# manycore-research/PlankAssembly

Hardware: AMD Instinct MI355X
Metric: train samples/sec (fwd+bwd+all-reduce+Adam), d_model=512 seq=1024 [value: bf16 MFMA, f32 accumulate / master weights; train.f32 / train.x3: the same step in exact f32 / f32 with bf16x3 products = the parity paths] (higher is better)
Workload: dtype bf16; 1 GPU; train_complete.yaml model d_model=512 H=8 dff=1024 6+6 post-norm layers, dropout 0.2, S=1024 (MAX_INPUT_LENGTH 1025), T=128, batch 16/GPU; global_batch=16, seq_len=1024, parallelism=dp1

## Files before the change

### plankassembly_amd/csrc/gemm.hip

```cpp
#include <stdlib.h>
#include <atomic>
#include <new>
#include <mutex>
#include <vector>
#include <type_traits>
#include <utility>
#include "pa_device.h"
#include <mutex>
#include <vector>
#include "../../include/plank_hip.h"
#include "gemm_common.h"

namespace {

constexpr int BM = 128, BN = 128, NT = 256;
__device__ __attribute__((aligned(16))) const uint32_t pa_zero16[4] = {0u, 0u, 0u, 0u};
typedef short s16x4 __attribute__((ext_vector_type(4)));

#ifdef PA_GEMM_TRACE
__device__ unsigned long long pa_trace[8192];
__device__ int pa_trace_n;
#define TR_DECL __shared__ unsigned long long tr_lds[1024]; int tr_n = 0
#define TR(tag) do { if (blockIdx.x == 0 && threadIdx.x == 0 && tr_n < 1022) { tr_lds[tr_n++] = (unsigned long long)(tag); tr_lds[tr_n++] = __builtin_amdgcn_s_memtime(); } } while (0)
#define TR_FLUSH do { if (blockIdx.x == 0 && threadIdx.x == 0) { for (int i_ = 0; i_ < tr_n; ++i_) pa_trace[i_] = tr_lds[i_]; pa_trace_n = tr_n; } } while (0)
// ... 1503 lines not shown
#ifndef PA_G3S_OLD
    u32x4 F[8];
#pragma unroll
    for (int s_ = 0; s_ < 4; ++s_) { PA_RD128(F[2 * s_], lds0 + fa_off + xs[s_]); PA_RD128(F[2 * s_ + 1], lds0 + fb_off + xs[s_]); }
#pragma unroll 1
    while (true) {
        const bool has_next = pending >= 2;
        if (has_next) wait_items(pending - 2);
        __builtin_amdgcn_s_barrier();
        if (cd_u < p.units) issue();
        {
            const uint32_t nst = lds0 + ((sc + 1) & (NSTG - 1)) * STAGE;
#pragma unroll
            for (int s_ = 0; s_ < 4; ++s_) {
                asm volatile("s_waitcnt lgkmcnt(6)" : "+v"(F[2 * s_]), "+v"(F[2 * s_ + 1]));
                acc = __builtin_amdgcn_mfma_f32_32x32x16_bf16(*reinterpret_cast<const bf16x8*>(&F[2 * s_ + 1]), *reinterpret_cast<const bf16x8*>(&F[2 * s_]), acc, 0, 0, 0);
                PA_RD128(F[2 * s_], nst + fa_off + xs[s_]); PA_RD128(F[2 * s_ + 1], nst + fb_off + xs[s_]);
            }
        }
        sc = (sc + 1) & (NSTG - 1);
        if (++cc_t >= nt) {
            PA_TR3(3);
            epilogue(cun);
#ifdef PA_GEMM_TRACE3
            PA_TR3(5);
            asm volatile("s_waitcnt vmcnt(0)" ::: "memory");
#endif
            PA_TR3(4);
            cc_u += ustride; cc_t = 0;
            if (cc_u < p.units) unit_of(cc_u, cun);
        }
        --pending;
        if (!has_next) break;
    }
    asm volatile("s_waitcnt lgkmcnt(0)" : "+v"(F[0]), "+v"(F[1]), "+v"(F[2]), "+v"(F[3]), "+v"(F[4]), "+v"(F[5]), "+v"(F[6]), "+v"(F[7]));
#else
    u32x4 F0[2], F1[2];
    frag(F0, lds0, 0);
    auto item = [&](auto HOT_) -> bool {
        constexpr bool HOT = decltype(HOT_)::value;
        const uint32_t st = lds0 + sc * STAGE;
        __builtin_amdgcn_s_barrier();
        if constexpr (!HOT) { if (cd_u < p.units) issue(); }
        wait_frag(F0); acc = __builtin_amdgcn_mfma_f32_32x32x16_bf16(*reinterpret_cast<const bf16x8*>(&F0[1]), *reinterpret_cast<const bf16x8*>(&F0[0]), acc, 0, 0, 0);
        frag(F1, st, 1); if constexpr (HOT) { fetch_q(sd, Q0{}); fetch_q(sd, Q1{}); }
        wait_frag(F1); acc = __builtin_amdgcn_mfma_f32_32x32x16_bf16(*reinterpret_cast<const bf16x8*>(&F1[1]), *reinterpret_cast<const bf16x8*>(&F1[0]), acc, 0, 0, 0);
        frag(F0, st, 2); if constexpr (HOT) { fetch_q(sd, Q2{}); fetch_q(sd, Q3{}); fetch_done(); sd = (sd + 1) & (NSTG - 1); ++cd_t; }
        wait_frag(F0); acc = __builtin_amdgcn_mfma_f32_32x32x16_bf16(*reinterpret_cast<const bf16x8*>(&F0[1]), *reinterpret_cast<const bf16x8*>(&F0[0]), acc, 0, 0, 0);
        frag(F1, st, 3);
        const bool has_next = HOT || pending >= 2;
        wait_frag(F1);
        if (has_next) {
            if constexpr (HOT) wait_items(2); else wait_items(pending - 2);
            __builtin_amdgcn_s_barrier();
            frag(F0, lds0 + ((sc + 1) & (NSTG - 1)) * STAGE, 0);
        }
        acc = __builtin_amdgcn_mfma_f32_32x32x16_bf16(*reinterpret_cast<const bf16x8*>(&F1[1]), *reinterpret_cast<const bf16x8*>(&F1[0]), acc, 0, 0, 0);
        sc = (sc + 1) & (NSTG - 1);
        if constexpr (HOT) { ++cc_t; return true; }
        else {
            if (++cc_t >= nt) {
                PA_TR3(3);
                epilogue(cun);
#ifdef PA_GEMM_TRACE3
                PA_TR3(5);
                asm volatile("s_waitcnt vmcnt(0)" ::: "memory");
#endif
                PA_TR3(4);
                cc_u += ustride; cc_t = 0;
                if (cc_u < p.units) unit_of(cc_u, cun);
            }
            --pending;
            return has_next;
        }
    };
#pragma unroll 1
    while (true) {
        int hot = (pending == 3 && cd_u == cc_u) ? (nt - cd_t - 1) : 0;
#pragma unroll 1
        for (; hot > 0; --hot) item(std::true_type{});
        if (!item(std::false_type{})) break;
    }
#endif
#undef PA_RD128
}

template <int FM, int FN>
__global__ __launch_bounds__(NT, 1) void gemm3w_kernel(GemmP p) {
    using T = bf16;
    constexpr int TBM = 64 * FM, TBN = 64 * FN;
    constexpr int RB = 128, NCH = 8;
    constexpr int A_BYTES = TBM * RB, B_BYTES = TBN * RB;
    constexpr int NLA = TBM * NCH / NT, NLB = TBN * NCH / NT, NLD = NLA + NLB;
    constexpr int NSTG = 3, STAGE = A_BYTES + B_BYTES, EPI = 32 * 32 * 4;
    static_assert(NSTG * STAGE + 4 * EPI <= 160 * 1024, "LDS budget");
    __shared__ __attribute__((aligned(256))) char smem[NSTG * STAGE + 4 * EPI];
    const int tid = threadIdx.x, lane = tid & 63;
    const int wave = __builtin_amdgcn_readfirstlane(tid >> 6);
    const int wm = wave >> 1, wn = wave & 1;
    const int half = lane >> 5;
    constexpr int esz = 2;
    f32x16 acc[FN][FM];
#pragma unroll
    for (int i = 0; i < FN; ++i)
#pragma unroll
        for (int j = 0; j < FM; ++j)
#pragma unroll
            for (int r = 0; r < 16; ++r) acc[i][j][r] = 0.f;

    uint32_t offA[NLA], offB[NLB];
    const char* kA = nullptr; const char* kB = nullptr;
    auto setup = [&](const Unit& un) {
        kA = reinterpret_cast<const char*>(p.A) + (size_t)un.b * p.sA * esz;
        kB = reinterpret_cast<const char*>(p.B) + (size_t)un.b * p.sB * esz;
        const int m0 = un.tile_m * TBM, n0 = un.tile_n * TBN;
#pragma unroll
        for (int i = 0; i < NLA; ++i) {
            const int pidx = tid + i * NT, row = pidx / NCH, ch = ((pidx % NCH) ^ (row / 2)) & (NCH - 1);
            offA[i] = (uint32_t)min(m0 + row, p.M - 1) * (uint32_t)(p.lda * esz) + ch * 16;
        }
#pragma unroll
        for (int i = 0; i < NLB; ++i) {
            const int pidx = tid + i * NT, row = pidx / NCH, ch = ((pidx % NCH) ^ (row / 2)) & (NCH - 1);
            offB[i] = (uint32_t)min(n0 + row, p.N - 1) * (uint32_t)(p.ldb * esz) + ch * 16;
        }
    };
    auto fetch_c = [&](int stage, auto C_) {
        constexpr int c = decltype(C_)::value;
        char* lx = smem + stage * STAGE + (c < NLA ? 0 : A_BYTES);
        constexpr int i = c < NLA ? c : c - NLA;
        const char* src = (c < NLA) ? kA + offA[i] : kB + offB[i];
        __builtin_amdgcn_global_load_lds((const __attribute__((address_space(1))) void*)src,
            (__attribute__((address_space(3))) void*)(lx + (i * NT + wave * 64) * 16), 16, 0, 0);
    };
    auto fetch_done = [&]() { kA += 64 * esz; kB += 64 * esz; };
    auto fetch_range = [&](int stage, auto LO_, auto HI_) {
        constexpr int LO = decltype(LO_)::value, HI = decltype(HI_)::value;
        static_for<LO, HI>([&](auto I_) { fetch_c(stage, I_); });
    };
    auto fetch = [&](int stage) {
        fetch_range(stage, std::integral_constant<int, 0>{}, std::integral_constant<int, NLD>{});
        fetch_done();
    };

    const uint32_t lds0 = (uint32_t)(uintptr_t)((__attribute__((address_space(3))) char*)smem);
    const int sw = ((lane & 31) >> 1) & 7;
    uint32_t xs[4];
#pragma unroll
    for (int s_ = 0; s_ < 4; ++s_) xs[s_] = (uint32_t)((((2 * s_ + half) ^ sw) & 7) << 4);
    const uint32_t fa_off = (wm * 32 * FM + (lane & 31)) * RB, fb_off = (wn * 32 * FN + (lane & 31)) * RB + A_BYTES;
#define PA_RD128O(dst, addr, OFF) asm volatile("ds_read_b128 %0, %1 offset:%2" : "=v"(dst) : "v"(addr), "n"(OFF))
    auto rd1 = [&](u32x4 (&f)[FM + FN], uint32_t st, int s_, auto W_) {
        constexpr int W = decltype(W_)::value;
        if constexpr (W < FM) { const uint32_t ad = st + fa_off + xs[s_]; PA_RD128O(f[W], ad, W * 32 * RB); }
        else { const uint32_t ad = st + fb_off + xs[s_]; PA_RD128O(f[W], ad, (W - FM) * 32 * RB); }
    };
    auto frag = [&](u32x4 (&f)[FM + FN], uint32_t st, int s_) {
        static_for<0, FM + FN>([&](auto I_) { rd1(f, st, s_, I_); });
    };
    auto wait_frag = [&](u32x4 (&f)[FM + FN]) {
        asm volatile("s_waitcnt lgkmcnt(0)" ::: "memory");
#pragma unroll
        for (int i = 0; i < FM + FN; ++i) asm volatile("" : "+v"(f[i]));
    };

    auto epilogue = [&](const Unit& un) {
// ... 926 lines not shown
                const size_t slab = (size_t)a->M * a->N * sizeof(float);
                if (hipMemsetAsync(static_cast<char*>(a->ws) + (size_t)got * slab, 0, (size_t)(want - got) * slab,
                                   reinterpret_cast<hipStream_t>(stream)) != hipSuccess) return PA_EINVAL;
            }
            return 0;
        }
        static const bool dbg_split = getenv("PA_SPLIT_DEBUG") && atoi(getenv("PA_SPLIT_DEBUG"));
        if (dbg_split) fprintf(stderr, "[pa_gemm x3 declined] M %d N %d K %d batch %d akc %d bkc %d lda %d ldb %d sA %lld sB %lld splitk %d aux %d ldaux %d\n",
                               a->M, a->N, a->K, a->batch, a->a_kcontig, a->b_kcontig, a->lda, a->ldb, (long long)a->sA, (long long)a->sB, a->splitk, a->aux ? 1 : 0, a->ldaux);
    }
    if (g_rec) { std::lock_guard<std::mutex> lk(g_rec_mu); if (g_rec) g_rec->push_back(*a); }
    if (a->M <= 0 || a->N <= 0 || a->K <= 0 || a->batch <= 0) return PA_EINVAL;
    if (a->in_dtype != PA_F32 && a->in_dtype != PA_BF16) return PA_EINVAL;
    if (a->out_dtype != PA_F32 && a->out_dtype != PA_BF16) return PA_EINVAL;
    if (a->drop_p < 0.f || a->drop_p >= 1.f) return PA_EINVAL;
    hipStream_t st = reinterpret_cast<hipStream_t>(stream);
    GemmP p;
    p.A = a->A; p.B = a->B; p.C = a->C; p.bias = a->bias; p.R = a->R; p.aux = a->aux;
    p.M = a->M; p.N = a->N; p.K = a->K;
    p.lda = a->lda; p.ldb = a->ldb; p.ldc = a->ldc; p.ldr = a->ldr; p.ldaux = a->ldaux;
    p.sA = a->sA; p.sB = a->sB; p.sC = a->sC; p.sR = a->sR; p.sAux = a->sAux; p.sBias = a->sBias;
    p.batch = a->batch;
    p.alpha = a->alpha; p.relu = a->relu; p.aux_scale = a->aux_scale;
    p.drop_thr = (uint32_t)((double)a->drop_p * 4294967296.0);
    p.drop_scale = (float)(1.0 / (1.0 - (double)p.drop_thr / 4294967296.0));
    p.drop_seed = a->drop_seed;
    p.out_dtype = a->out_dtype;
    p.ln_u = nullptr; p.ln_gamma = nullptr; p.ln_beta = nullptr; p.ln_y = nullptr; p.ldy = 0; p.ln_eps = 0.f;
    p.c_lp = a->C_lp; p.ldc_lp = a->ldc_lp; p.ln_zf = nullptr; p.ldzf = 0; p.ln_y_f32 = 0;
    if (a->C_lp && (a->out_dtype != PA_F32 || a->ldc_lp < a->N || a->ldc_lp % 4 || (reinterpret_cast<uintptr_t>(a->C_lp) & 7))) return PA_EINVAL;
    static const int dbg_bk = getenv("PA_GEMM_BK") ? atoi(getenv("PA_GEMM_BK")) : 64;
    const bool bk32 = a->in_dtype == PA_BF16 && dbg_bk == 32;
    const int BK = a->in_dtype == PA_BF16 ? (bk32 ? 32 : 64) : 16;
    const int nt = (a->K + BK - 1) / BK;
    int splitk = a->splitk > 1 ? a->splitk : 1;
    if (splitk > nt) splitk = nt;
    splitk = (nt + (nt + splitk - 1) / splitk - 1) / ((nt + splitk - 1) / splitk);
    if (splitk > 1 && !a->ws) return PA_EINVAL;
    p.splitk = splitk;
    p.tiles_per_slice = (nt + splitk - 1) / splitk;
    p.tiles_m = (a->M + BM - 1) / BM;
    p.tiles_n = (a->N + BN - 1) / BN;
    p.plain_order = p.tiles_m < 8;
    p.tiles_m_pad = p.plain_order ? p.tiles_m : (p.tiles_m + 7) / 8 * 8;
    p.units = p.tiles_m_pad * p.tiles_n * a->batch * splitk;
    GemmP pk = p;
    if (splitk > 1) { pk.C = a->ws; pk.ldc = a->N; }
    {
        const int osz = (splitk > 1 || a->out_dtype == PA_F32) ? 4 : 2, isz = a->in_dtype == PA_BF16 ? 2 : 4;
        auto ok = [](const void* q, long long ld, long long sb, int esz) {
            return !q || (((reinterpret_cast<uintptr_t>(q) * 1) % (4 * esz) == 0) && (ld % 4 == 0) && (sb % 4 == 0));
        };
        pk.vec_ok = ok(pk.C, pk.ldc, splitk > 1 ? (long long)a->M * a->N : a->sC, osz) && ok(a->R, a->ldr, a->sR, osz) &&
                    ok(a->aux, a->ldaux, a->sAux, isz) && ok(a->bias, 4, a->sBias, 4);
    }
    const int cus = cus_for_gemm();
    static const int dbg_noglds = getenv("PA_GEMM_NOGLDS") ? atoi(getenv("PA_GEMM_NOGLDS")) : 0;
    static const int dbg_grid = getenv("PA_GEMM_GRID") ? atoi(getenv("PA_GEMM_GRID")) :
                                (getenv("PA_GEMM_NST") && atoi(getenv("PA_GEMM_NST")) == 1 ? 1024 : (bk32 ? 768 : 512));
    static const int dbg_bits = getenv("PA_GEMM_DBG") ? atoi(getenv("PA_GEMM_DBG")) : 0;
    pk.dbg = dbg_bits; p.dbg = dbg_bits;
    const int pair_cap = dbg_grid > 0 ? (dbg_grid / 256) * cus + dbg_grid % 256 : 0;
    int grid_x = (pair_cap > 0 && pk.units > pair_cap) ? pair_cap : pk.units;
    dim3 grid(grid_x);
    const bool glds = ((a->K % BK) == 0 || (!a->a_kcontig && !a->b_kcontig && a->in_dtype == PA_BF16 && !bk32)) && !dbg_noglds;
    int rc;
    static const int use_v3 = getenv("PA_GEMM_V3") ? atoi(getenv("PA_GEMM_V3")) : 1;
    const bool v3_layout_ok = (a->a_kcontig && a->b_kcontig) ? (a->K % 64 == 0) : ((!a->a_kcontig || a->K % 64 == 0) && (!a->b_kcontig || a->K % 64 == 0));
    const int valid_units = p.tiles_m * p.tiles_n * a->batch * splitk;
    const bool go_v3 = use_v3 && (valid_units <= 256 || use_v3 == 2) && a->in_dtype == PA_BF16 && !bk32 && !dbg_noglds && is_aligned<bf16>(a) && v3_layout_ok;
    static const int use_small = getenv("PA_GEMM_SMALL") ? atoi(getenv("PA_GEMM_SMALL")) : 1;
    static const int small_max = getenv("PA_GEMM_SMALL_MAX") ? atoi(getenv("PA_GEMM_SMALL_MAX")) : 128;
    static const int small_max_k512 = getenv("PA_GEMM_SMALL_MAX_K512") ? atoi(getenv("PA_GEMM_SMALL_MAX_K512")) : 192;
    const bool go_small = go_v3 && use_small && a->a_kcontig && a->b_kcontig && splitk == 1 && a->K % 64 == 0 &&
                          (valid_units <= small_max || (valid_units <= small_max_k512 && a->K <= 512));
    static const int use_wide = getenv("PA_GEMM_WIDE") ? atoi(getenv("PA_GEMM_WIDE")) : 2;
    const long long wide_tiles = (long long)((a->M + 127) / 128) * ((a->N + 255) / 256) * a->batch;
    const bool go_wide = use_v3 && use_wide && (use_wide == 1 || wide_tiles <= cus) && a->in_dtype == PA_BF16 && !bk32 && !dbg_noglds &&
                         is_aligned<bf16>(a) && a->a_kcontig && a->b_kcontig && splitk == 1 && a->K % 64 == 0 && a->N >= 1024 && valid_units > 256;
    static const int use_tall = getenv("PA_GEMM_TALL") ? atoi(getenv("PA_GEMM_TALL")) : 0;
    const int tall_units = ((a->M + 191) / 192) * ((a->N + 127) / 128) * a->batch;
    const bool go_tall = use_v3 && use_tall && !go_wide && a->in_dtype == PA_BF16 && !bk32 && !dbg_noglds && is_aligned<bf16>(a) && a->a_kcontig &&
                         a->b_kcontig && splitk == 1 && a->K % 64 == 0 && valid_units > 256 && tall_units <= cus;
    static const int use_skinny = getenv("PA_GEMM_SKINNY") ? atoi(getenv("PA_GEMM_SKINNY")) : 2;
    static const int skinny_rows = getenv("PA_GEMM_SKINNY_ROWS") ? atoi(getenv("PA_GEMM_SKINNY_ROWS")) : 512;
    static const int skinny_rows32 = getenv("PA_GEMM_SKINNY_ROWS_F32") ? atoi(getenv("PA_GEMM_SKINNY_ROWS_F32"))
                                     : getenv("PA_GEMM_SKINNY_ROWS") ? atoi(getenv("PA_GEMM_SKINNY_ROWS")) : 2048;
    const int sk_ch = a->in_dtype == PA_BF16 ? 512 : 256;
    const bool go_skinny = use_skinny && (a->in_dtype == PA_F32 || use_skinny >= 2) && a->a_kcontig && a->b_kcontig && splitk == 1 &&
                           a->batch == 1 && a->M <= (a->in_dtype == PA_F32 ? skinny_rows32 : skinny_rows) && a->K % sk_ch == 0 && !a->aux && a->drop_p == 0.f && !dbg_noglds &&
                           (a->in_dtype == PA_BF16 ? is_aligned<bf16>(a) : is_aligned<float>(a));
    static const int use_big = getenv("PA_GEMM_BIG") ? atoi(getenv("PA_GEMM_BIG")) : 0;
    static const int big_minm = getenv("PA_GEMM_BIG_MINM") ? atoi(getenv("PA_GEMM_BIG_MINM")) : 4096;
    static const int big_minn = getenv("PA_GEMM_BIG_MINN") ? atoi(getenv("PA_GEMM_BIG_MINN")) : 256;
    const bool go_big = use_big && !go_skinny && a->in_dtype == PA_BF16 && !dbg_noglds && is_aligned<bf16>(a) && a->a_kcontig && a->b_kcontig &&
                        splitk == 1 && a->K % 64 == 0 && a->M >= big_minm && a->N >= big_minn;
    if (go_big) {
        if (g_rec) { std::lock_guard<std::mutex> lk(g_rec_mu); if (g_rec && g_rec_kind) g_rec_kind->push_back(PA_GEMM_KIND_BIG); if (g_rec && g_rec_group) g_rec_group->push_back(-1); }
        static const int force_tn = getenv("PA_GEMM_BIG_TN") ? atoi(getenv("PA_GEMM_BIG_TN")) : 0;
        int tn = a->N >= 1024 ? 256 : 128;
        const int tm8 = (a->M + 255) / 256;
        if (use_big >= 2) {
            long best = -1;
            for (int w : {256, 192, 128}) {
                const long blocks = (long)tm8 * ((a->N + w - 1) / w) * a->batch;
                const long rounds = (blocks + cus - 1) / cus;
                const long cost = rounds * w * 1000 + ((a->N + w - 1) / w * w - a->N);
                if (best < 0 || cost < best) { best = cost; tn = w; }
            }
        }
        if (force_tn == 256 || force_tn == 192 || force_tn == 128) tn = force_tn;
        GemmP pb = pk;
        pb.tiles_m = tm8; pb.tiles_n = (a->N + tn - 1) / tn;
        pb.plain_order = pb.tiles_m < 8;
        pb.tiles_m_pad = pb.plain_order ? pb.tiles_m : (pb.tiles_m + 7) / 8 * 8;
        pb.units = pb.tiles_m_pad * pb.tiles_n * a->batch;
        const int gb = pb.units < cus ? pb.units : cus;
        if (tn == 256) PA_LAUNCH((gemm8_kernel<4, 2, 2, 4, 64, 2>), dim3(gb), dim3(512), 0, st, pb);
        else if (tn == 192) PA_LAUNCH((gemm8_kernel<4, 2, 2, 3, 64, 2>), dim3(gb), dim3(512), 0, st, pb);
        else PA_LAUNCH((gemm8_kernel<4, 2, 2, 2, 64, 2>), dim3(gb), dim3(512), 0, st, pb);
        return 0;
    }
    if (a->C_lp && !go_skinny) return PA_EINVAL;
    if (go_skinny) {
        if (g_rec) { std::lock_guard<std::mutex> lk(g_rec_mu); if (g_rec && g_rec_kind) g_rec_kind->push_back(PA_GEMM_KIND_SKINNY); if (g_rec && g_rec_group) g_rec_group->push_back(-1); }
        GemmP ps = pk;
        ps.tiles_m = (a->M + SK_T - 1) / SK_T; ps.tiles_n = (a->N + SK_T - 1) / SK_T;
        const dim3 gsk(ps.tiles_m * ps.tiles_n);
        if (a->in_dtype == PA_BF16) PA_LAUNCH((gemm_skinny_kernel<bf16, false>), gsk, dim3(256), 0, st, ps);
        else PA_LAUNCH((gemm_skinny_kernel<float, false>), gsk, dim3(256), 0, st, ps);
        return 0;
    }
    if (g_rec) { std::lock_guard<std::mutex> lk(g_rec_mu); if (g_rec && g_rec_kind) g_rec_kind->push_back((go_wide || go_tall) ? PA_GEMM_KIND_WIDE : (go_small ? PA_GEMM_KIND_SMALL : (go_v3 ? PA_GEMM_KIND_RING : PA_GEMM_KIND_PAIR))); if (g_rec && g_rec_group) g_rec_group->push_back(-1); }
    if (go_wide) {
        GemmP pw = pk;
        pw.tiles_m = (a->M + 127) / 128; pw.tiles_n = (a->N + 255) / 256;
        pw.tiles_m_pad = (pw.tiles_m + 7) / 8 * 8; pw.plain_order = 0;
        pw.units = pw.tiles_m_pad * pw.tiles_n * a->batch;
        const int gw = pw.units < cus ? pw.units : cus;
        PA_LAUNCH((gemm3w_kernel<2, 4>), dim3(gw), dim3(NT), 0, st, pw);
        return 0;
    }
    if (go_tall) {
        GemmP pw = pk;
        pw.tiles_m = (a->M + 191) / 192; pw.tiles_n = (a->N + 127) / 128;
        pw.plain_order = pw.tiles_m < 8;
        pw.tiles_m_pad = pw.plain_order ? pw.tiles_m : (pw.tiles_m + 7) / 8 * 8;
        pw.units = pw.tiles_m_pad * pw.tiles_n * a->batch;
        const int gw = pw.units < cus ? pw.units : cus;
        PA_LAUNCH((gemm3w_kernel<3, 2>), dim3(gw), dim3(NT), 0, st, pw);
        return 0;
    }
    if (go_small) {
        GemmP ps = pk;
        ps.tiles_m = (a->M + 63) / 64; ps.tiles_n = (a->N + 63) / 64; ps.tiles_m_pad = ps.tiles_m; ps.plain_order = 1;
        ps.units = ps.tiles_m * ps.tiles_n * a->batch;
        const int gs = ps.units < 2 * cus ? ps.units : 2 * cus;
        PA_LAUNCH(gemm3s_kernel, dim3(gs), dim3(NT), 0, st, ps);
        rc = 0;
    } else
    if (go_v3) {
        const int g3 = pk.units < cus ? pk.units : cus;
        if (a->a_kcontig && a->b_kcontig) PA_LAUNCH((gemm3_kernel<true, true, GemmP>), dim3(g3), dim3(NT), 0, st, pk);
        else if (a->a_kcontig) PA_LAUNCH((gemm3_kernel<true, false, GemmP>), dim3(g3), dim3(NT), 0, st, pk);
        else if (a->b_kcontig) PA_LAUNCH((gemm3_kernel<false, true, GemmP>), dim3(g3), dim3(NT), 0, st, pk);
        else PA_LAUNCH((gemm3_kernel<false, false, GemmP>), dim3(g3), dim3(NT), 0, st, pk);
        rc = 0;
    } else
    if (a->in_dtype == PA_BF16) {
        if (bk32) rc = launch_layout<bf16, 32, 3>(pk, a->a_kcontig, a->b_kcontig, is_aligned<bf16>(a), glds, grid, st);
        else rc = launch_layout<bf16, 64, 2>(pk, a->a_kcontig, a->b_kcontig, is_aligned<bf16>(a), glds, grid, st);
    } else {
        rc = launch_layout<float, 16, 2>(pk, a->a_kcontig, a->b_kcontig, is_aligned<float>(a), glds, grid, st);
    }
    if (rc) return rc;
    if (splitk > 1 && a->splitk_defer) {
        if (a->out_dtype != PA_F32 || a->bias || a->R || a->aux || a->relu || a->drop_p > 0.f || a->alpha != 1.f || a->batch != 1) return PA_EINVAL;
        return 0;
    }
    if (splitk > 1) {
        size_t total = (size_t)a->batch * a->M * a->N;
        int blocks = (int)((total + 255) / 256);
        if (blocks > 2048) blocks = 2048;
        if (a->in_dtype == PA_BF16)
            PA_LAUNCH(splitk_reduce_kernel<bf16>, dim3(blocks), dim3(256), 0, st, p, (const float*)a->ws);
        else
            PA_LAUNCH(splitk_reduce_kernel<float>, dim3(blocks), dim3(256), 0, st, p, (const float*)a->ws);
    }
    return 0;
}

namespace {
template <typename TW>
__global__ __launch_bounds__(256) void ln_fold_weights_kernel(TW* Wf, float* u, float* v, const float* W, const float* bias,
                                                              const float* gamma, const float* beta, int N, int K) {
    __shared__ float red[2][4];
    const int n = blockIdx.x;
    float su = 0.f, sv = 0.f;
    for (int k = threadIdx.x; k < K; k += 256) {
        const float w = W[(size_t)n * K + k];
        const TW wf = (TW)(w * gamma[k]);
        Wf[(size_t)n * K + k] = wf;
        su += (float)wf;
        sv += w * beta[k];
    }
    su = wave_sum(su); sv = wave_sum(sv);
    if ((threadIdx.x & 63) == 0) { red[0][threadIdx.x >> 6] = su; red[1][threadIdx.x >> 6] = sv; }
    __syncthreads();
    if (threadIdx.x == 0) {
        u[n] = (red[0][0] + red[0][1]) + (red[0][2] + red[0][3]);
        v[n] = (bias ? bias[n] : 0.f) + (red[1][0] + red[1][1]) + (red[1][2] + red[1][3]);
    }
}
}
extern "C" int pa_ln_fold_weights(void* Wf, float* u, float* v, const float* W, const float* bias, const float* gamma,
                                  const float* beta, int32_t N, int32_t K, void* stream) {
    if (!Wf || !u || !v || !W || !gamma || !beta || N <= 0 || K <= 0) return PA_EINVAL;
    PA_LAUNCH(ln_fold_weights_kernel<bf16>, dim3(N), dim3(256), 0, reinterpret_cast<hipStream_t>(stream), (bf16*)Wf, u, v, W, bias, gamma, beta, N, K);
    return 0;
}
extern "C" int pa_ln_fold_weights_f32(float* Wf, float* u, float* v, const float* W, const float* bias, const float* gamma,
                                      const float* beta, int32_t N, int32_t K, void* stream) {
    if (!Wf || !u || !v || !W || !gamma || !beta || N <= 0 || K <= 0) return PA_EINVAL;
    PA_LAUNCH(ln_fold_weights_kernel<float>, dim3(N), dim3(256), 0, reinterpret_cast<hipStream_t>(stream), Wf, u, v, W, bias, gamma, beta, N, K);
    return 0;
}
extern "C" int pa_gemm_norm_a(const pa_gemm_args* a, const pa_gemm_norm_ext* x, void* stream) {
    if (!a || !x || !a->A || !a->B || !a->C || !a->bias || !x->u || a->M <= 0 || a->N <= 0 || a->K <= 0) return PA_EINVAL;
    if ((a->in_dtype != PA_BF16 && a->in_dtype != PA_F32) || (a->out_dtype != PA_BF16 && a->out_dtype != PA_F32) || !a->a_kcontig || !a->b_kcontig) return PA_EINVAL;
    if (a->in_dtype == PA_F32) {
        static const int sk_rows32 = getenv("PA_GEMM_SKINNY_ROWS") ? atoi(getenv("PA_GEMM_SKINNY_ROWS")) : 512;
        if (a->batch != 1 || a->splitk > 1 || a->R || a->aux || a->drop_p != 0.f || a->N % 32) return PA_ESHAPE;
        if (!x->zf || a->K != 512 || a->M > sk_rows32 || a->out_dtype != PA_F32 || (x->y && (!x->y_f32 || a->N < a->K))) return PA_ESHAPE;
        if (x->y && (!x->gamma || !x->beta || x->ldy < a->K || x->ldy % 4 || (reinterpret_cast<uintptr_t>(x->y) & 15))) return PA_EINVAL;
        if (!is_aligned<float>(a) || x->ldzf < a->K || x->ldzf % 4 || (reinterpret_cast<uintptr_t>(x->zf) & 15)) return PA_EALIGN;
        GemmP p = GemmP();
        p.A = a->A; p.B = a->B; p.C = a->C; p.bias = a->bias;
        p.M = a->M; p.N = a->N; p.K = a->K; p.lda = a->lda; p.ldb = a->ldb; p.ldc = a->ldc;
        p.batch = 1; p.alpha = a->alpha; p.relu = a->relu; p.aux_scale = 1.f; p.drop_scale = 1.f; p.out_dtype = PA_F32; p.splitk = 1;
        p.tiles_m = (a->M + SK_T - 1) / SK_T; p.tiles_n = (a->N + SK_T - 1) / SK_T;
        p.vec_ok = ((reinterpret_cast<uintptr_t>(a->C) & 15) == 0 && a->ldc % 4 == 0 && (reinterpret_cast<uintptr_t>(a->bias) & 15) == 0 &&
                    (reinterpret_cast<uintptr_t>(x->u) & 15) == 0 && (!x->y || ((reinterpret_cast<uintptr_t>(x->gamma) & 15) == 0 &&
                                                                          (reinterpret_cast<uintptr_t>(x->beta) & 15) == 0))) ? 1 : 0;
        if (!p.vec_ok) return PA_EALIGN;
        p.ln_u = x->u; p.ln_gamma = x->gamma; p.ln_beta = x->beta; p.ln_y = x->y; p.ldy = x->ldy; p.ln_eps = x->eps;
        p.ln_zf = x->zf; p.ldzf = x->ldzf; p.ln_y_f32 = 1;
        PA_LAUNCH((gemm_skinny_kernel<float, true>), dim3(p.tiles_m * p.tiles_n), dim3(256), 0, reinterpret_cast<hipStream_t>(stream), p);
        return 0;
    }
// ... 648 lines not shown
```

### plankassembly_amd/csrc/gemm_common.h

```cpp
#pragma once
#include <type_traits>
#include <utility>
#include "pa_device.h"
#include "../../include/plank_hip.h"

namespace {

struct GemmP {
    const void* A; const void* B; void* C;
    const float* bias; const void* R; const void* aux;
    int M, N, K;
    int lda, ldb, ldc, ldr, ldaux;
    long long sA, sB, sC, sR, sAux, sBias;
    int batch;
    float alpha; int relu; float aux_scale;
    uint32_t drop_thr; float drop_scale; uint32_t drop_seed;
    int out_dtype;
    int splitk, tiles_per_slice;
    int tiles_m, tiles_n, tiles_m_pad, units;
    int vec_ok;
    int plain_order;
    int dbg;
    const float* ln_u; const float* ln_gamma; const float* ln_beta; void* ln_y; int ldy; float ln_eps;
    void* c_lp; int ldc_lp;
    const float* ln_zf; int ldzf; int ln_y_f32;
};

struct Unit { int tile_m, tile_n, b, z, t_begin, t_end; };

template <int LO, int... I, typename F>
__device__ __forceinline__ void static_for_impl(F&& f, std::integer_sequence<int, I...>) { (f(std::integral_constant<int, LO + I>{}), ...); }
template <int LO, int HI, typename F>
__device__ __forceinline__ void static_for(F&& f) { static_for_impl<LO>(f, std::make_integer_sequence<int, (HI > LO ? HI - LO : 0)>{}); }


}
```

Measured before the change: 3495 samples/s.

## Add two-blocks-per-CU persistent bf16 GEMM kernel for large-unit fallback cases

Adds a new persistent GEMM kernel (gemm3p) with two LDS stages and launch bounds allowing two workgroups per CU. It uses magic-number division for tile decoding, software-pipelined ds_read fragments interleaved with MFMAs, and an epilogue that prefetches residual/aux data. The kernel is selected by default for contiguous bf16 GEMMs that previously fell back to the generic layout kernels when valid units exceed 256. It aims to hide load latency through higher occupancy and overlapped fetches, at the cost of less LDS pipelining depth per block and a new, complex code path.

```diff
diff --git a/plankassembly_amd/csrc/gemm.hip b/plankassembly_amd/csrc/gemm.hip
--- a/plankassembly_amd/csrc/gemm.hip
+++ b/plankassembly_amd/csrc/gemm.hip
@@ -1609,6 +1609,330 @@
         if (!item(std::false_type{})) break;
     }
 #endif
+#undef PA_RD128
+}
+
+__global__ __launch_bounds__(NT, 2) void gemm3p_kernel(GemmP p) {
+    using T = bf16;
+    using TL = Tile<bf16, 64>;
+    constexpr int NSTG = 2, STAGE = 2 * TL::TILE_BYTES, EPI = 16 * 256;
+    __shared__ __attribute__((aligned(256))) char smem[NSTG * STAGE + 4 * EPI];
+    const int tid = threadIdx.x, lane = tid & 63;
+    const int wave = __builtin_amdgcn_readfirstlane(tid >> 6);
+    const int wm = wave >> 1, wn = wave & 1;
+    const int half = lane >> 5;
+    constexpr int esz = 2;
+
+    f32x16 acc[2][2];
+#pragma unroll
+    for (int i = 0; i < 2; ++i)
+#pragma unroll
+        for (int j = 0; j < 2; ++j)
+#pragma unroll
+            for (int r = 0; r < 16; ++r) acc[i][j][r] = 0.f;
+
+    const int ustride = gridDim.x, nt = p.K / 64, per_z = p.tiles_m_pad * p.tiles_n;
+    auto udiv = [](int n, unsigned long long mag) { return (int)(((unsigned long long)(uint32_t)n * mag) >> 32); };
+    auto decode = [&](int u, Unit& un) -> bool {
+        const int z = udiv(u, p.mag_z), r = u - z * per_z;
+        if (p.plain_order) {
+            un.tile_m = udiv(r, p.mag_n);
+            un.tile_n = r - un.tile_m * p.tiles_n;
+        } else {
+            const int i = r >> 3, q = udiv(i, p.mag_n);
+            un.tile_n = i - q * p.tiles_n;
+            un.tile_m = q * 8 + (r & 7);
+        }
+        un.b = z; un.z = z; un.t_begin = 0; un.t_end = nt;
+        return un.tile_m < p.tiles_m;
+    };
+    auto seek = [&](int u, Unit& un) -> int {
+        while (u < p.units && !decode(u, un)) u += ustride;
+        return u;
+    };
+
+    uint32_t offA[TL::NLD], offB[TL::NLD];
+    const char* kA = nullptr; const char* kB = nullptr;
+    auto setup = [&](const Unit& un) {
+        const int m0 = un.tile_m * BM, n0 = un.tile_n * BN;
+#pragma unroll
+        for (int i = 0; i < TL::NLD; ++i) {
+            const int pidx = tid + i * NT, row = pidx / TL::NCH, ch = ((pidx % TL::NCH) ^ (row / TL::RPB)) & (TL::NCH - 1);
+            offA[i] = (uint32_t)min(m0 + row, p.M - 1) * (uint32_t)(p.lda * esz) + ch * 16;
+            offB[i] = (uint32_t)min(n0 + row, p.N - 1) * (uint32_t)(p.ldb * esz) + ch * 16;
+        }
+        kA = reinterpret_cast<const char*>(p.A) + (size_t)un.b * p.sA * esz;
+        kB = reinterpret_cast<const char*>(p.B) + (size_t)un.b * p.sB * esz;
+    };
+    auto fetch = [&](int stage) {
+        char* la = smem + stage * STAGE;
+        char* lb = la + TL::TILE_BYTES;
+#pragma unroll
+        for (int i = 0; i < TL::NLD; ++i)
+            __builtin_amdgcn_global_load_lds((const __attribute__((address_space(1))) void*)(kA + offA[i]),
+                (__attribute__((address_space(3))) void*)(la + (i * NT + wave * 64) * 16), 16, 0, 0);
+#pragma unroll
+        for (int i = 0; i < TL::NLD; ++i)
+            __builtin_amdgcn_global_load_lds((const __attribute__((address_space(1))) void*)(kB + offB[i]),
+                (__attribute__((address_space(3))) void*)(lb + (i * NT + wave * 64) * 16), 16, 0, 0);
+        kA += TL::BK * esz; kB += TL::BK * esz;
+    };
+
+    const uint32_t lds0 = (uint32_t)(uintptr_t)((__attribute__((address_space(3))) char*)smem);
+    const int sw = ((lane & 31) >> 1) & 7;
+    uint32_t xs[4];
+#pragma unroll
+    for (int s_ = 0; s_ < 4; ++s_) xs[s_] = (uint32_t)((((2 * s_ + half) ^ sw) & 7) << 4);
+    const uint32_t fa_off = (wm * 64 + (lane & 31)) * TL::RB, fb_off = (wn * 64 + (lane & 31)) * TL::RB + TL::TILE_BYTES;
+#define PA_RD128(dst, addr, OFF) asm volatile("ds_read_b128 %0, %1 offset:%2" : "=v"(dst) : "v"(addr), "n"(OFF))
+    auto rd1 = [&](u32x4 (&f)[4], uint32_t st, auto S_, auto W_) {
+        constexpr int S = decltype(S_)::value, W = decltype(W_)::value, i = W & 1;
+        if constexpr (W < 2) { const uint32_t ad = st + fa_off + xs[S]; PA_RD128(f[W], ad, i * 32 * TL::RB); }
+        else { const uint32_t ad = st + fb_off + xs[S]; PA_RD128(f[W], ad, i * 32 * TL::RB); }
+    };
+    using W0 = std::integral_constant<int, 0>; using W1 = std::integral_constant<int, 1>;
+    using W2 = std::integral_constant<int, 2>; using W3 = std::integral_constant<int, 3>;
+    auto wait_frag = [&](u32x4 (&f)[4]) {
+        __builtin_amdgcn_sched_barrier(0);
+        asm volatile("s_waitcnt lgkmcnt(0)" : "+v"(f[0]), "+v"(f[1]), "+v"(f[2]), "+v"(f[3]));
+    };
+    auto step = [&](u32x4 (&fc)[4], u32x4 (&fn)[4], uint32_t stn, auto SN_) {
+        wait_frag(fc);
+        mma16B<T>(acc[0][0], fc[2], fc[0]); rd1(fn, stn, SN_, W0{});
+        mma16B<T>(acc[0][1], fc[2], fc[1]); rd1(fn, stn, SN_, W1{});
+        mma16B<T>(acc[1][0], fc[3], fc[0]); rd1(fn, stn, SN_, W2{});
+        mma16B<T>(acc[1][1], fc[3], fc[1]); rd1(fn, stn, SN_, W3{});
+    };
+
+    f32x4 ubias = {0.f, 0.f, 0.f, 0.f};
+    auto load_bias = [&](const Unit& un) {
+        ubias = f32x4{0.f, 0.f, 0.f, 0.f};
+        if (p.bias) {
+            const int n = un.tile_n * BN + wn * 64 + (lane & 15) * 4;
+            const float* bp = p.bias + (size_t)un.b * p.sBias;
+            if (p.vec_ok && n + 3 < p.N) ubias = *reinterpret_cast<const f32x4*>(bp + n);
+            else { for (int e = 0; e < 4; ++e) if (n + e < p.N) ubias[e] = bp[n + e]; }
+        }
+    };
+    u32x2 pre[16];
+    int pre_kind = 0;
+    auto prefetch_epi = [&](const Unit& un) {
+        pre_kind = 0;
+        if (p.out_dtype == PA_F32 || (p.R == nullptr && p.aux == nullptr)) return;
+        if (!(p.vec_ok && un.tile_n * BN + wn * 64 + 64 <= p.N)) return;
+        const bool use_r = p.R != nullptr;
+        pre_kind = use_r ? 1 : 2;
+        const char* base = use_r ? reinterpret_cast<const char*>(p.R) + (size_t)un.b * p.sR * 2
+                                 : reinterpret_cast<const char*>(p.aux) + (size_t)un.b * p.sAux * 2;
+        const uint32_t ld2 = (uint32_t)(use_r ? p.ldr : p.ldaux) * 2u;
+        const int mw = un.tile_m * BM + wm * 64, n = un.tile_n * BN + wn * 64 + (lane & 15) * 4, rsub = lane >> 4;
+#pragma unroll
+        for (int j = 0; j < 16; ++j)
+            pre[j] = *reinterpret_cast<const u32x2*>(base + ((uint32_t)min(mw + j * 4 + rsub, p.M - 1) * ld2 + (uint32_t)n * 2u));
+    };
+    auto widen = [](const u32x2& u) { f32x4 r; r[0] = bf16_lo(u[0]); r[1] = bf16_hi(u[0]); r[2] = bf16_lo(u[1]); r[3] = bf16_hi(u[1]); return r; };
+
+    auto epilogue = [&](const Unit& un) {
+        char* stage = smem + NSTG * STAGE + wave * EPI;
+        const size_t cbase = (size_t)un.b * p.sC;
+        const int mw = un.tile_m * BM + wm * 64, nw = un.tile_n * BN + wn * 64;
+        const int chunk = lane & 15, rsub = lane >> 4;
+        const int n = nw + chunk * 4;
+        const bool out_f32 = p.out_dtype == PA_F32;
+        const bool has_bias = p.bias != nullptr, has_aux = p.aux != nullptr, has_res = p.R != nullptr, has_drop = p.drop_thr != 0;
+        const bool fast = p.vec_ok && (nw + 64 <= p.N);
+        const f32x4 bias = has_bias ? ubias : f32x4{0.f, 0.f, 0.f, 0.f};
+        constexpr int NIT = 4;
+        static_for<0, 4>([&](auto P_) {
+            constexpr int P = decltype(P_)::value, tm = P >> 1, h = P & 1;
+            {
+                const int lrow = (lane & 31) - 16 * h;
+                if (lrow >= 0 && lrow < 16) {
+#pragma unroll
+                    for (int tn = 0; tn < 2; ++tn)
+#pragma unroll
+                        for (int g4 = 0; g4 < 4; ++g4) {
+                            f32x4 v;
+#pragma unroll
+                            for (int e = 0; e < 4; ++e) v[e] = acc[tn][tm][4 * g4 + e];
+                            const int ch = tn * 8 + 2 * g4 + half;
+                            *reinterpret_cast<f32x4*>(stage + lrow * 256 + ((ch ^ lrow) << 4)) = v;
+                        }
+                }
+            }
+            f32x4 x[NIT];
+            const int mp = mw + 16 * P + rsub;
+#pragma unroll
+            for (int it = 0; it < NIT; ++it) {
+                const int lr = it * 4 + rsub;
+                x[it] = *reinterpret_cast<const f32x4*>(stage + lr * 256 + ((chunk ^ lr) << 4));
+            }
+            if (fast) {
+                f32x4 res[NIT], gate[NIT];
+                if (has_res) {
+                    if (pre_kind == 1) {
+#pragma unroll
+                        for (int it = 0; it < NIT; ++it) res[it] = widen(pre[4 * P + it]);
+                    } else if (out_f32) {
+#pragma unroll
+                        for (int it = 0; it < NIT; ++it)
+                            res[it] = ld4<float>(reinterpret_cast<const float*>(p.R) + (size_t)un.b * p.sR + (size_t)min(mp + it * 4, p.M - 1) * p.ldr + n);
+                    } else {
+#pragma unroll
+                        for (int it = 0; it < NIT; ++it)
+                            res[it] = ld4<bf16>(reinterpret_cast<const bf16*>(p.R) + (size_t)un.b * p.sR + (size_t)min(mp + it * 4, p.M - 1) * p.ldr + n);
+                    }
+                }
+                if (has_aux) {
+                    if (pre_kind == 2) {
+#pragma unroll
+                        for (int it = 0; it < NIT; ++it) gate[it] = widen(pre[4 * P + it]);
+                    } else {
+#pragma unroll
+                        for (int it = 0; it < NIT; ++it)
+                            gate[it] = ld4<T>(reinterpret_cast<const T*>(p.aux) + (size_t)un.b * p.sAux + (size_t)min(mp + it * 4, p.M - 1) * p.ldaux + n);
+                    }
+                }
+#pragma unroll
+                for (int it = 0; it < NIT; ++it)
+#pragma unroll
+                    for (int e = 0; e < 4; ++e) x[it][e] = x[it][e] * p.alpha + bias[e];
+                if (p.relu) {
+#pragma unroll
+                    for (int it = 0; it < NIT; ++it)
+#pragma unroll
+                        for (int e = 0; e < 4; ++e) x[it][e] = fmaxf(x[it][e], 0.f);
+                }
+                if (has_aux) {
+#pragma unroll
+                    for (int it = 0; it < NIT; ++it)
+#pragma unroll
+                        for (int e = 0; e < 4; ++e) x[it][e] = gate[it][e] > 0.f ? x[it][e] * p.aux_scale : 0.f;
+                }
+                if (has_drop) {
+#pragma unroll
+                    for (int it = 0; it < NIT; ++it)
+#pragma unroll
+                        for (int e = 0; e < 4; ++e)
+                            x[it][e] = drop_keep_rc(p.drop_seed, (uint32_t)(un.b * p.M + mp + it * 4), (uint32_t)(n + e), p.drop_thr) ? x[it][e] * p.drop_scale : 0.f;
+                }
+                if (has_res) {
+#pragma unroll
+                    for (int it = 0; it < NIT; ++it)
+#pragma unroll
+                        for (int e = 0; e < 4; ++e) x[it][e] += res[it][e];
+                }
+                const bool interior = mw + 16 * P + 16 <= p.M;
+                const size_t co0 = cbase + (size_t)mp * p.ldc + n, rstep = (size_t)4 * p.ldc;
+                if (out_f32) {
+                    float* cp = reinterpret_cast<float*>(p.C) + co0;
+                    if (interior) {
+#pragma unroll
+                        for (int it = 0; it < NIT; ++it) *reinterpret_cast<f32x4*>(cp + it * rstep) = x[it];
+                    } else {
+#pragma unroll
+                        for (int it = 0; it < NIT; ++it) if (mp + it * 4 < p.M) *reinterpret_cast<f32x4*>(cp + it * rstep) = x[it];
+                    }
+                } else {
+                    bf16* cp = reinterpret_cast<bf16*>(p.C) + co0;
+                    if (interior) {
+#pragma unroll
+                        for (int it = 0; it < NIT; ++it) st4<bf16>(cp + it * rstep, x[it]);
+                    } else {
+#pragma unroll
+                        for (int it = 0; it < NIT; ++it) if (mp + it * 4 < p.M) st4<bf16>(cp + it * rstep, x[it]);
+                    }
+                }
+            } else {
+#pragma unroll 1
+                for (int it = 0; it < NIT; ++it) {
+                    const int m = mp + it * 4;
+                    if (m >= p.M) continue;
+                    for (int e = 0; e < 4; ++e) {
+                        if (n + e >= p.N) continue;
+                        float y = x[it][e] * p.alpha + bias[e];
+                        if (p.relu) y = fmaxf(y, 0.f);
+                        if (has_aux) {
+                            const float g = ld1(reinterpret_cast<const T*>(p.aux) + (size_t)un.b * p.sAux + (size_t)m * p.ldaux + n + e);
+                            y = g > 0.f ? y * p.aux_scale : 0.f;
+                        }
+                        if (has_drop) y = drop_keep_rc(p.drop_seed, (uint32_t)(un.b * p.M + m), (uint32_t)(n + e), p.drop_thr) ? y * p.drop_scale : 0.f;
+                        if (has_res) {
+                            const size_t ro = (size_t)un.b * p.sR + (size_t)m * p.ldr + n + e;
+                            y += out_f32 ? reinterpret_cast<const float*>(p.R)[ro] : (float)reinterpret_cast<const bf16*>(p.R)[ro];
+                        }
+                        const size_t co = cbase + (size_t)m * p.ldc + n + e;
+                        if (out_f32) reinterpret_cast<float*>(p.C)[co] = y;
+                        else reinterpret_cast<bf16*>(p.C)[co] = (bf16)y;
+                    }
+                }
+            }
+        });
+        asm volatile("" :: "v"(bias[0]), "v"(bias[1]), "v"(bias[2]), "v"(bias[3]));
+#pragma unroll
+        for (int j = 0; j < 16; ++j) asm volatile("" :: "v"(pre[j]));
+#pragma unroll
+        for (int i = 0; i < 2; ++i)
+#pragma unroll
+            for (int j = 0; j < 2; ++j)
+#pragma unroll
+                for (int r = 0; r < 16; ++r) acc[i][j][r] = 0.f;
+    };
+
+    Unit cun, dun;
+    int cc_u = seek(blockIdx.x, cun), cc_t = 0;
+    if (cc_u >= p.units) return;
+    int cd_u = cc_u, cd_t = 0;
+    dun = cun;
+    setup(dun);
+    load_bias(cun);
+    int sd = 0, pending = 0;
+    auto issue = [&]() {
+        fetch(sd);
+        sd ^= 1;
+        ++pending;
+        if (++cd_t >= nt) { cd_u = seek(cd_u + ustride, dun); cd_t = 0; if (cd_u < p.units) setup(dun); }
+    };
+    issue();
+    if (cd_u < p.units) {
+        issue();
+        __builtin_amdgcn_s_waitcnt(0x0F78);
+    } else {
+        __builtin_amdgcn_s_waitcnt(0x0F70);
+    }
+    __builtin_amdgcn_s_barrier();
+    using S0 = std::integral_constant<int, 0>; using S1 = std::integral_constant<int, 1>;
+    using S2 = std::integral_constant<int, 2>; using S3 = std::integral_constant<int, 3>;
+    u32x4 F0[4], F1[4];
+    rd1(F0, lds0, S0{}, W0{}); rd1(F0, lds0, S0{}, W1{}); rd1(F0, lds0, S0{}, W2{}); rd1(F0, lds0, S0{}, W3{});
+    int sc = 0;
+#pragma unroll 1
+    while (true) {
+        const uint32_t st = lds0 + sc * STAGE, stn = lds0 + (sc ^ 1) * STAGE;
+        const bool last_k = cc_t + 1 >= nt;
+        if (last_k) prefetch_epi(cun);
+        step(F0, F1, st, S1{});
+        step(F1, F0, st, S2{});
+        step(F0, F1, st, S3{});
+        const bool has_next = pending >= 2;
+        if (has_next) {
+            __builtin_amdgcn_s_waitcnt(0x0F70);
+            __builtin_amdgcn_s_barrier();
+        }
+        step(F1, F0, stn, S0{});
+        if (cd_u < p.units) {
+            __builtin_amdgcn_s_barrier();
+            issue();
+        }
+        sc ^= 1;
+        --pending;
+        if (last_k) {
+            epilogue(cun);
+            if (has_next) { cc_u = seek(cc_u + ustride, cun); cc_t = 0; load_bias(cun); }
+        } else ++cc_t;
+        if (!has_next) break;
+    }
+    asm volatile("s_waitcnt lgkmcnt(0)" : "+v"(F0[0]), "+v"(F0[1]), "+v"(F0[2]), "+v"(F0[3]));
 #undef PA_RD128
 }
 
@@ -2701,6 +3025,11 @@
     const int tall_units = ((a->M + 191) / 192) * ((a->N + 127) / 128) * a->batch;
     const bool go_tall = use_v3 && use_tall && !go_wide && a->in_dtype == PA_BF16 && !bk32 && !dbg_noglds && is_aligned<bf16>(a) && a->a_kcontig &&
                          a->b_kcontig && splitk == 1 && a->K % 64 == 0 && valid_units > 256 && tall_units <= cus;
+    static const int use_pair3 = getenv("PA_GEMM_PAIR3") ? atoi(getenv("PA_GEMM_PAIR3")) : 1;
+    static const bool nst_forced = getenv("PA_GEMM_NST") && atoi(getenv("PA_GEMM_NST")) != 0;
+    const bool go_pair3 = use_pair3 && !nst_forced && !dbg_bits && a->in_dtype == PA_BF16 && !bk32 && !dbg_noglds && is_aligned<bf16>(a) &&
+                          a->a_kcontig && a->b_kcontig && splitk == 1 && a->K % 64 == 0 &&
+                          (unsigned long long)p.units * (unsigned long long)(p.tiles_m_pad * p.tiles_n) < (1ull << 32);
     static const int use_skinny = getenv("PA_GEMM_SKINNY") ? atoi(getenv("PA_GEMM_SKINNY")) : 2;
     static const int skinny_rows = getenv("PA_GEMM_SKINNY_ROWS") ? atoi(getenv("PA_GEMM_SKINNY_ROWS")) : 512;
     static const int skinny_rows32 = getenv("PA_GEMM_SKINNY_ROWS_F32") ? atoi(getenv("PA_GEMM_SKINNY_ROWS_F32"))
@@ -2784,6 +3113,12 @@
         else if (a->a_kcontig) PA_LAUNCH((gemm3_kernel<true, false, GemmP>), dim3(g3), dim3(NT), 0, st, pk);
         else if (a->b_kcontig) PA_LAUNCH((gemm3_kernel<false, true, GemmP>), dim3(g3), dim3(NT), 0, st, pk);
         else PA_LAUNCH((gemm3_kernel<false, false, GemmP>), dim3(g3), dim3(NT), 0, st, pk);
+        rc = 0;
+    } else
+    if (go_pair3) {
+        pk.mag_z = (1ull << 32) / (unsigned long long)(pk.tiles_m_pad * pk.tiles_n) + 1ull;
+        pk.mag_n = (1ull << 32) / (unsigned long long)pk.tiles_n + 1ull;
+        PA_LAUNCH(gemm3p_kernel, grid, dim3(NT), 0, st, pk);
         rc = 0;
     } else
     if (a->in_dtype == PA_BF16) {
diff --git a/plankassembly_amd/csrc/gemm_common.h b/plankassembly_amd/csrc/gemm_common.h
--- a/plankassembly_amd/csrc/gemm_common.h
+++ b/plankassembly_amd/csrc/gemm_common.h
@@ -24,6 +24,7 @@
     const float* ln_u; const float* ln_gamma; const float* ln_beta; void* ln_y; int ldy; float ln_eps;
     void* c_lp; int ldc_lp;
     const float* ln_zf; int ldzf; int ln_y_f32;
+    unsigned long long mag_z, mag_n;
 };
 
 struct Unit { int tile_m, tile_n, b, z, t_begin, t_end; };
```

New measurement: 3540 samples/s (median of 6 runs). 1.3% higher.
